# Kebii/MikuDance

Hardware: AMD Instinct MI355X
Metric: frames/sec (768x768, 16f, 20 DDIM steps) (higher is better)
Workload: dtype f16; 1 GPU; configs[1]: 768x768, 16-frame clip, 20 DDIM steps, fp16, reference_unet + denoising_unet + motion_module, CFG 3.5, one clip per GPU per step; parallelism=dp1, input_staging=rank-local (every rank stages its own clip in HBM before the timed region), reference_reuse=True, queues=1, weights=random-init SD-1.5 geometry (N(0,1/fan_in), seeds 1234/4321), width=full

## Files before the change

include/mdance_hip.h:

```cpp
#ifndef MDANCE_HIP_H
#define MDANCE_HIP_H
#include <stddef.h>
#ifdef __cplusplus
extern "C" {
#endif

#define MD_ACT_NONE 0
#define MD_ACT_SILU 1
#define MD_ACT_RELU 2
#define MD_ACT_GEGLU 3
#define MD_ACT_QUICKGELU 4

int md_version(void);
const char* md_last_error(void);

int md_gemm_f16(const void* A, int lda, const void* W, void* C, int ldc, int M, int N, int K, const void* bias,
                const void* residual, int ldr, const void* rowadd, int ldra, int rows_per_group, int act,
                int transpose_out, void* stream);

int md_conv3x3_nhwc_f16(const void* X, const void* W, void* Y, int ldy, int B, int Hin, int Win, int Cin, int Cout,
                        int stride, int upsample, const void* bias, const void* residual, int ldr,
                        const void* rowadd, int ldra, int rows_per_group, int act, void* stream);

int md_conv3x3_pad_nhwc_f16(const void* X, const void* W, void* Y, int ldy, int B, int Hin, int Win, int Cin, int Cout,
                            int stride, int upsample, int pad_lo, const void* bias, const void* residual, int ldr,
                            const void* rowadd, int ldra, int rows_per_group, int act, void* stream);

int md_conv_nhwc_f16(const void* X, int ldx, const void* W, void* Y, int ldy, int B, int Hin, int Win, int Cin, int Cout, int kw,
                     int stride, int upsample, int pad_lo, const void* bias, const void* residual, int ldr, const void* rowadd,
                     int ldra, int rows_per_group, int act, void* stream);

int md_softmax_rows_f16(void* x, int ldx, int rows, int cols, float scale, void* stream);

size_t md_groupnorm_workspace_bytes(int B, int HW, int C, int G);
int md_groupnorm_nhwc_f16(const void* x, void* y, const void* gamma, const void* beta, int B, int HW, int C, int G,
                          float eps, int silu, void* workspace, size_t ws_bytes, void* stream);

int md_groupnorm_ld_nhwc_f16(const void* x, int ldx, void* y, const void* gamma, const void* beta, int B, int HW, int C, int G,
                             float eps, int silu, void* workspace, size_t ws_bytes, void* stream);

int md_layernorm_f16(const void* x, void* y, void* y2, const void* gamma, const void* beta, const void* add, int M,
                     int C, float eps, int add_mode, int add_row_begin, int rows_per_frame, int frames, void* stream);

int md_groupnorm_plan(int B, int HW, int C, int G, int ldx, int x_align16, int table, int* threads, int* R, int* slab, int* nslab);

int md_layernorm_plan(int M, int C);

int md_gemm_ln_plan(int M, int N, int K, int act, int epi);
int md_gemm_ln_f16(const void* A, int lda, const void* Wf, const float* sc, void* C, int ldc, int M, int N, int K, float eps,
                   const void* rowadd, int ldra, int rows_per_group, int act, void* stream);

int md_groupnorm_table_f16(const void* x, int ldx, const void* gamma, const void* beta, int B, int HW, int C, int G, float eps,
                           float* table, void* workspace, size_t ws_bytes, void* stream);
int md_gemm_affine_plan(int M, int N, int K, int rows_per_image);
int md_gemm_affine_f16(const void* A, int lda, const float* table, int rows_per_image, const void* W, void* C, int ldc, int M, int N,
                       int K, const void* bias, void* stream);

int md_instnorm_spade_f16(const void* x, const void* gamma_beta, void* y, int B, int HW, int C, float eps,
                          void* stream);

int md_instnorm_spade_ld_f16(const void* x, int ldx, const void* gamma_beta, void* y, int B, int HW, int C, float eps,
                             void* stream);

int md_attention_fwd_f16(const void* Q, int ldq, const void* K, int ldk, const void* Vt, int ldvt, void* O, int ldo,
                         const int* kv_index, int B, int H, int D, int Lq, int Lk, int kv_stride, float scale,
                         void* stream);

int md_attention_plan(int D, int Lq, int Lk, int kv_stride, int ldvt, int vt_align16);

int md_temporal_attention_fwd_f16(const void* Q, int ldq, const void* K, int ldk, const void* V, int ldv, void* O,
                                  int ldo, int NB, int F, int HW, int H, int D, float scale, void* stream);

int md_temporal_attention_plan(int NB, int F, int HW, int H, int D, int aligned16, int* hg, int* pb);

int md_pack_nhwc_f16(const void* src, int src_is_f32, void* dst, int N, int F, long sB, long sF, long sC, long sY,
                     long sX, int c_begin, int c_count, int Cpad, int Ho, int Wo, int Hin, int Win, void* stream);
int md_unpack_nhwc_f16(const void* src, int ldc, void* dst, int dst_is_f32, int N, int F, long sB, long sF, long sC,
                       long sY, long sX, int C, int Ho, int Wo, void* stream);

int md_concat_channels_f16(const void* a, int Ca, const void* b, int Cb, void* out, long M, void* stream);

int md_window_accumulate(const void* pred, void* noise_sum, void* counter, const int* window, int f, int Ftot, int HW,
                         int halves, void* stream);

int md_window_accumulate_weighted(const void* pred, void* noise_sum, void* counter, const int* window, const float* weights, int f,
                                  int Ftot, int HW, int halves, void* stream);

int md_cfg_ddim_step(void* latents, const void* noise_sum, const void* counter, int Ftot, int HW, int halves,
                     float guidance, float alpha_t, float alpha_prev, void* stream);
// ... 84 lines not shown
```

mikudance_amd/_lib.py:

```python
import ctypes
import os
from ctypes import c_char_p, c_float, c_int, c_long, c_size_t, c_void_p

_HERE = os.path.dirname(os.path.abspath(__file__))
LIB_PATH = os.path.join(_HERE, "libmdance_hip.so")

P = c_void_p
SIGNATURES = {
    "md_version": (c_int, []),
    "md_last_error": (c_char_p, []),
    "md_gemm_f16": (c_int, [P, c_int, P, P, c_int, c_int, c_int, c_int, P, P, c_int, P, c_int, c_int, c_int, c_int, P]),
    "md_conv3x3_nhwc_f16": (c_int, [P, P, P, c_int, c_int, c_int, c_int, c_int, c_int, c_int, c_int, P, P, c_int, P, c_int,
                                    c_int, c_int, P]),
    "md_conv3x3_pad_nhwc_f16": (c_int, [P, P, P, c_int, c_int, c_int, c_int, c_int, c_int, c_int, c_int, c_int, P, P, c_int, P,
                                        c_int, c_int, c_int, P]),
    "md_conv_nhwc_f16": (c_int, [P, c_int, P, P, c_int, c_int, c_int, c_int, c_int, c_int, c_int, c_int, c_int, c_int, P, P, c_int, P,
                                 c_int, c_int, c_int, P]),
    "md_set_cu_limit": (c_int, [c_int]),
    "md_gemm_plan": (c_int, [c_int, c_int, c_int, c_int, c_int, c_int, c_int]),
    "md_conv3x3_plan": (c_int, [c_int, c_int, c_int, c_int, c_int, c_int, c_int, c_int, c_int]),
    "md_gemm_plan_call": (c_int, [P, c_int, P, P, c_int, c_int, c_int, c_int, P, P, c_int, P, c_int, c_int, c_int, c_int,
                                  ctypes.POINTER(c_int), ctypes.POINTER(c_int)]),
    "md_conv_plan_call": (c_int, [P, c_int, P, P, c_int, c_int, c_int, c_int, c_int, c_int, c_int, c_int, c_int, c_int, P, P, c_int, P,
                                  c_int, c_int, c_int]),
    "md_softmax_rows_f16": (c_int, [P, c_int, c_int, c_int, c_float, P]),
    "md_groupnorm_workspace_bytes": (c_size_t, [c_int, c_int, c_int, c_int]),
    "md_groupnorm_nhwc_f16": (c_int, [P, P, P, P, c_int, c_int, c_int, c_int, c_float, c_int, P, c_size_t, P]),
    "md_groupnorm_ld_nhwc_f16": (c_int, [P, c_int, P, P, P, c_int, c_int, c_int, c_int, c_float, c_int, P, c_size_t, P]),
    "md_instnorm_spade_ld_f16": (c_int, [P, c_int, P, P, c_int, c_int, c_int, c_float, P]),
    "md_layernorm_f16": (c_int, [P, P, P, P, P, P, c_int, c_int, c_float, c_int, c_int, c_int, c_int, P]),
    "md_groupnorm_plan": (c_int, [c_int, c_int, c_int, c_int, c_int, c_int, c_int] + [ctypes.POINTER(c_int)] * 4),
    "md_layernorm_plan": (c_int, [c_int, c_int]),
    "md_gemm_ln_plan": (c_int, [c_int, c_int, c_int, c_int, c_int]),
    "md_gemm_ln_f16": (c_int, [P, c_int, P, P, P, c_int, c_int, c_int, c_int, c_float, P, c_int, c_int, c_int, P]),
    "md_groupnorm_table_f16": (c_int, [P, c_int, P, P, c_int, c_int, c_int, c_int, c_float, P, P, c_size_t, P]),
    "md_gemm_affine_plan": (c_int, [c_int, c_int, c_int, c_int]),
    "md_gemm_affine_f16": (c_int, [P, c_int, P, c_int, P, P, c_int, c_int, c_int, c_int, P, P]),
    "md_instnorm_spade_f16": (c_int, [P, P, P, c_int, c_int, c_int, c_float, P]),
    "md_attention_fwd_f16": (c_int, [P, c_int, P, c_int, P, c_int, P, c_int, P, c_int, c_int, c_int, c_int, c_int, c_int,
                                     c_float, P]),
    "md_attention_plan": (c_int, [c_int, c_int, c_int, c_int, c_int, c_int]),
    "md_temporal_attention_fwd_f16": (c_int, [P, c_int, P, c_int, P, c_int, P, c_int, c_int, c_int, c_int, c_int, c_int,
                                              c_float, P]),
    "md_temporal_attention_plan": (c_int, [c_int, c_int, c_int, c_int, c_int, c_int, ctypes.POINTER(c_int), ctypes.POINTER(c_int)]),
    "md_pack_nhwc_f16": (c_int, [P, c_int, P, c_int, c_int, c_long, c_long, c_long, c_long, c_long, c_int, c_int, c_int,
                                 c_int, c_int, c_int, c_int, P]),
    "md_unpack_nhwc_f16": (c_int, [P, c_int, P, c_int, c_int, c_int, c_long, c_long, c_long, c_long, c_long, c_int, c_int,
                                   c_int, P]),
    "md_concat_channels_f16": (c_int, [P, c_int, P, c_int, P, c_long, P]),
    "md_window_accumulate": (c_int, [P, P, P, P, c_int, c_int, c_int, c_int, P]),
    "md_window_accumulate_weighted": (c_int, [P, P, P, P, P, c_int, c_int, c_int, c_int, P]),
    "md_cfg_ddim_step": (c_int, [P, P, P, c_int, c_int, c_int, c_float, c_float, c_float, P]),
    "md_cfg_ddim_step_eta": (c_int, [P, P, P, P, c_int, c_int, c_int, c_float, c_float, c_float, c_float, P]),
    "md_cfg_multistep_step": (c_int, [P, P, P, P, P, c_int, c_int, c_int, c_float, c_float, c_float, c_float, c_float, c_float, c_float, P]),
    "md_cfg_rescale_workspace_bytes": (c_size_t, [c_int, c_int]),
    "md_cfg_guidance_rescale": (c_int, [P, P, c_int, c_int, c_int, c_float, c_float, P, c_size_t, P, P]),
    "md_cfg_ddim_step_scaled": (c_int, [P, P, P, P, P, c_int, c_int, c_int, c_float, c_float, c_float, c_float, P]),
    "md_cfg_multistep_step_scaled": (c_int, [P, P, P, P, P, P, c_int, c_int, c_int, c_float, c_float, c_float, c_float, c_float, c_float,
                                             c_float, P]),
    "md_cfg_apg_workspace_bytes": (c_size_t, [c_int, c_int]),
    "md_cfg_apg_prepare": (c_int, [P, P, P, P, c_int, c_int, c_int, c_float, c_float, c_float, c_float, c_float, P, c_size_t, P, P]),
    "md_cfg_ddim_step_apg": (c_int, [P, P, P, P, P, P, c_int, c_int, c_int, c_float, c_float, c_float, c_float, P]),
    "md_cfg_multistep_step_apg": (c_int, [P, P, P, P, P, P, P, c_int, c_int, c_int, c_float, c_float, c_float, c_float, c_float, c_float,
                                          c_float, P]),
    "md_cfg_ddim_step_pag": (c_int, [P, P, P, P, P, c_int, c_int, c_int, c_float, c_float, c_float, c_float, c_float, P]),
    "md_cfg_multistep_step_pag": (c_int, [P, P, P, P, P, P, c_int, c_int, c_int, c_float, c_float, c_float, c_float, c_float, c_float, c_float,
                                          c_float, P]),
    "md_cfg_unipc_step": (c_int, [P, P, P, P, c_int, c_int, c_int, c_float, P, P]),
    "md_cfg_unipc_step_scaled": (c_int, [P, P, P, P, P, c_int, c_int, c_int, c_float, P, P]),
    "md_cfg_unipc_step_apg": (c_int, [P, P, P, P, P, P, c_int, c_int, c_int, c_float, P, P]),
# ... 80 lines not shown
```

mikudance_amd/blocks.py:

```python
from dataclasses import dataclass

import torch
from torch import nn

from . import ops, packing

GROUPS = 32
HEADS = 8


class _Packed(nn.Module):

    def __init__(self):
        super().__init__()
        self._pk = None

    def _apply(self, fn, *a, **k):
        self._pk = None
        return super()._apply(fn, *a, **k)

    def _load_from_state_dict(self, *a, **k):
        self._pk = None
        return super()._load_from_state_dict(*a, **k)

# ... 109 lines not shown
class _GEGLU(nn.Module):
    def __init__(self, dim):
        super().__init__()
        self.proj = Linear(dim, dim * 8)


class FeedForward(nn.Module):

    def __init__(self, dim):
        super().__init__()
        self.net = nn.ModuleList([_GEGLU(dim), nn.Identity(), Linear(dim * 4, dim)])


def _pack_ff(ff, dev, pk, prefix="ff"):
    w, b = packing.geglu_weight(ff.net[0].proj.weight, ff.net[0].proj.bias, dev)
    pk[prefix + "1"], pk[prefix + "1b"] = w, b
    pk[prefix + "2"], pk[prefix + "2b"] = packing.linear_weight(ff.net[2].weight, dev), packing.vec(ff.net[2].bias, dev)


FUSE_NORMS = __import__("os").environ.get("MD_FUSE_NORMS", "1") != "0"


def ln_linear(pk, h, norm, lin, bias=None, rowadd=None, rows_per_group=0, act=ops.ACT_NONE, eps=1e-5):
    M, K = h.shape
    w = pk[lin]
    if FUSE_NORMS and ops.gemm_ln_plan(M, w.shape[0], K, act, rowadd is not None, a=h):
        fk = lin + ":ln"
        if fk not in pk:
            pk[fk] = packing.ln_fold(w, None if bias is None else pk[bias], pk[norm + "w"], pk[norm + "b"])
        wf, sc = pk[fk]
        return ops.gemm_ln(h, wf, sc, eps=eps, rowadd=rowadd, rows_per_group=rows_per_group, act=act)
    n = ops.layernorm(h, pk[norm + "w"], pk[norm + "b"], eps=eps)
    return ops.gemm(n, w, bias=None if bias is None else pk[bias], rowadd=rowadd, rows_per_group=rows_per_group, act=act)


def gn_linear(x, gamma, beta, eps, w, bias):
    B, C = x.shape[0], x.shape[-1]
    M = x.numel() // C
    if FUSE_NORMS and ops.gemm_affine_plan(M, w.shape[0], C, M // B, x=x):
        return ops.gemm_affine(x, ops.groupnorm_table(x, gamma, beta, GROUPS, eps), w, bias=bias)
    return ops.gemm(tokens(ops.groupnorm(x, gamma, beta, GROUPS, eps)), w, bias=bias)


def _run_ff(pk, h, norm, prefix="ff"):
    g = ln_linear(pk, h, norm, prefix + "1", bias=prefix + "1b", act=ops.ACT_GEGLU)
    return ops.gemm(g, pk[prefix + "2"], bias=pk[prefix + "2b"], residual=h)


class CrossContext:

    def __init__(self, ctx, index, lk, lpad, zero_frames=0):
        self.ctx, self.index, self.lk, self.lpad = ctx, index, lk, lpad
        self.zero_frames = zero_frames
        self.root = self
        self._slices = {}

    def rows(self, lo, hi):
        s = self._slices.get((lo, hi))
        if s is None:
            s = CrossContext(self.ctx, self.index[lo:hi].contiguous(), self.lk, self.lpad, zero_frames=max(0, min(self.zero_frames, hi) - lo))
            s.root = self.root
            self._slices[(lo, hi)] = s
        return s


ZERO_CONTEXT_SKIP = True
# ... 15 lines not shown

    @property
    def perturbed(self):
        return self.identity is not None or self.blur is not None


PLAIN = SelfAttnCall()


class TransformerBlock(_Packed):

    def __init__(self, dim, ctx_dim, heads=HEADS, kind="2d"):
        super().__init__()
        self.dim, self.heads, self.kind = dim, heads, kind
        self.norm1 = Affine(dim)
        self.attn1 = Attention(dim)
        self.norm2 = Affine(dim)
        self.attn2 = Attention(dim, ctx_dim)
        self.norm3 = Affine(dim)
        self.ff = FeedForward(dim)
        self.bank = []
        self.ref_mode = None
        self.ref_cfg = False
        self.stop_after_bank = False
        self._kv_cache = None

    def _pack(self, dev):
        L, V = packing.linear_weight, packing.vec
        a1, a2 = self.attn1, self.attn2
        pk = {f"n{i}w": V(n.weight, dev) for i, n in ((1, self.norm1), (2, self.norm2), (3, self.norm3))}
        pk.update({f"n{i}b": V(n.bias, dev) for i, n in ((1, self.norm1), (2, self.norm2), (3, self.norm3))})
        pk["q1"], pk["k1"], pk["v1"] = L(a1.to_q.weight, dev), L(a1.to_k.weight, dev), L(a1.to_v.weight, dev)
        pk["qk1"] = torch.cat([pk["q1"], pk["k1"]], 0).contiguous()
        pk["o1"], pk["o1b"] = L(a1.to_out[0].weight, dev), V(a1.to_out[0].bias, dev)
        pk["q2"], pk["k2"], pk["v2"] = L(a2.to_q.weight, dev), L(a2.to_k.weight, dev), L(a2.to_v.weight, dev)
        pk["o2"], pk["o2b"] = L(a2.to_out[0].weight, dev), V(a2.to_out[0].bias, dev)
        _pack_ff(self.ff, dev, pk)
        self._kv_cache = None
        return pk

    def context_kv(self, cross):
        if self._kv_cache is None or self._kv_cache[0] is not cross.root:
            pk = self.packed()
            self._kv_cache = (cross.root, ops.gemm(cross.ctx, pk["k2"]), ops.gemm(cross.ctx, pk["v2"], transpose_out=True), {})
        return self._kv_cache[1:]

    def _self_attention(self, pk, n, kv, B, L, grid, sigma, pool, tile):
        C, H = self.dim, self.heads
        t, shift = tile or (1, None)
        th, tw = (grid[0] // t, grid[1] // t) if grid is not None else (None, None)
        Bt, Lt = (B, L) if tile is None else (B * t * t, th * tw)
        pad = None if tile is None else (Lt + 7) // 8 * 8

        def order(x, stride=None):
            return x if tile is None else ops.token_tile(x, B, grid[0], grid[1], t, shift, tile_stride=stride)[0]

        if n is kv and pool is None and sigma is None and pad in (None, Lt):
            src = order(n)
            qk = ops.gemm(src, pk["qk1"])
            q, k, Lk, stride = qk[:, :C], qk[:, C:], Lt, None
        else:
            if sigma is not None:
                q = order(ops.token_blur(ops.gemm(n, pk["q1"]), B, grid[0], grid[1], sigma))
            else:
                q = ops.gemm(order(n), pk["q1"])
            if pool is None:
                src, Lk, stride = order(kv, pad), Lt, pad
            else:
                src, Lk, stride = ops.token_pool(order(kv), Bt, th, tw, pool[0], pool[1])
            k = ops.gemm(src, pk["k1"])
        vt = ops.gemm(src, pk["v1"], transpose_out=True)
        a = ops.attention(q, k, vt, Bt, H, C // H, Lt, Lk, kv_stride=stride)
        return a if tile is None else ops.token_untile(a, B, grid[0], grid[1], t, shift)

    def forward(self, h, B, L, cross, sa=PLAIN, grid=None):
        pk = self.packed()
        C, H = self.dim, self.heads
        D = C // H
        if sa.perturbed and self.ref_mode == "write":
            raise ValueError("TransformerBlock: a perturbed evaluation is a call of its own: not a bank write")
        identity = sa.identity is not None and any(self is b for b in sa.identity)
        sigma = sa.blur[1] if sa.blur is not None and any(self is b for b in sa.blur[0]) else None
        pool = None if sa.pool is None or identity else sa.pool.get(self)
        tile = None if sa.tile is None or identity else sa.tile.get(self)
        if (sigma is not None or pool is not None or tile is not None) and (grid is None or grid[0] * grid[1] != L):
            raise ValueError(f"TransformerBlock: grid {grid} does not hold L = {L} tokens")
        M = h.shape[0]
        if self.ref_mode != "read" or len(self.bank) != 1 or (self.ref_cfg and sa.half == 0):
            begin = None
        elif sa.perturbed or sa.half == 1 or not self.ref_cfg:
            begin = 0
        else:
            begin = M // 2
        if begin is None:
            n = kv = ops.layernorm(h, pk["n1w"], pk["n1b"])
            if self.ref_mode == "write":
                self.bank.append(n.view(B, L, C))
                if self.stop_after_bank:
                    return h
        else:
            b2 = self.bank[0].reshape(-1, C)
            if (self.ref_cfg or sa.perturbed) and b2.shape[0] == 2 * (M - begin):
                b2 = b2[M - begin:]
            assert b2.shape[0] == M - begin, (b2.shape, M)
# ... 168 lines not shown
```

mikudance_amd/csrc/gemm.hip:

```cpp
#include "common.h"
#include <stdlib.h>
#include <algorithm>


enum { ACT_NONE = 0, ACT_SILU = 1, ACT_RELU = 2, ACT_GEGLU = 3, ACT_QUICKGELU = 4 };

struct GemmParams {
  const half_t* A;
  const half_t* W;
  half_t* C;
  const half_t* bias;
  const half_t* residual;
  const half_t* rowadd;
  int lda, ldc, ldr, ldra;
  int M, N, K;
  int rows_per_group;
  int act;
  int transpose_out;
  int bias_rows;
  int Hin, Win, Cin, Hout, Wout, stride, upsample, pad;
  int ldx;
  int kw;
  int tiles_n, tiles_total;
  int tiles_m, group_m;
// ... 564 lines not shown
  MD_CHECK_LAUNCH("md_gemm_ln");
  return MD_OK;
}

extern "C" int md_gemm_affine_plan(int M, int N, int K, int rows_per_image) {
  return rows_per_image > 0 && rows_per_image % 16 == 0 && M % rows_per_image == 0 && ws_fused_shape(M, N, K, K, N);
}

extern "C" int md_gemm_affine_f16(const void* A, int lda, const float* table, int rows_per_image, const void* W, void* C, int ldc, int M, int N,
                                  int K, const void* bias, void* stream) {
  MD_CHECK_ARG(rows_per_image > 0 && rows_per_image % 16 == 0 && M % rows_per_image == 0 && ws_fused_shape(M, N, K, lda, ldc),
               "md_gemm_affine: no fused kernel for M=%d N=%d K=%d rows_per_image=%d (ask md_gemm_affine_plan first)", M, N, K, rows_per_image);
  MD_CHECK_ARG(al16(A) && al16(W) && al16(C) && al16(table) && al16(bias), "md_gemm_affine: operands must be 16-byte aligned");
  MD_CHECK_ARG(A != C, "md_gemm_affine: in place is not supported");
  WsParams p = {};
  p.A = (const half_t*)A; p.W = (const half_t*)W; p.C = (half_t*)C; p.bias = (const half_t*)bias;
  p.lda = lda; p.ldc = ldc; p.M = M; p.N = N; p.rows_per_group = 1;
  p.aff = table; p.rows_per_image = rows_per_image;
  p.groups = N / 320; ws_streams(p);
  hipStream_t st = (hipStream_t)stream;
  if (p.groups > 1) launch_ws_fused<2, false, PRO_AFF>(p, st);
  else launch_ws_fused<1, false, PRO_AFF>(p, st);
  MD_CHECK_LAUNCH("md_gemm_affine");
  return MD_OK;
}

static bool ws_eligible(const GemmParams& p) {
  if (p.act != ACT_NONE || p.transpose_out || p.M < 32768 || p.M % 16) return false;
  const bool k320 = p.K == 320 && p.N % 320 == 0 && p.N / 320 <= 8;
  const bool k640 = p.K == 640 && p.N % 128 == 0 && p.N / 128 <= 16;
  if (!k320 && !k640) return false;
  if (p.lda % 8 || p.ldc % 8 || (p.residual && p.ldr % 8) || (p.rowadd && p.ldra % 8)) return false;
  return al16(p.A) && al16(p.W) && al16(p.C) && al16(p.bias) && al16(p.residual) && al16(p.rowadd);
}

struct SpTile {
  int code, bm, bn;
  double t_k;
  int pin;
  bool (*eligible)(const GemmParams&);
  bool (*resm)(const GemmParams&);
  void (*launch)(GemmParams&, bool resm, int ncu, hipStream_t);
};
template <bool CONV, bool GEGLU, int MT, int NT>
static SpTile sp_tile(double t_k, int pin) {
  return {100 + 10 * MT + NT, 64 * MT, 64 * NT, t_k, pin, sp_eligible<CONV, GEGLU, NT>, GEGLU ? nullptr : sp_resm<MT, NT>,
          launch_sp<CONV, GEGLU, NT, MT>};
}
enum { T135, T134, T124, T142, T132, T144, SP_TILES };
static const SpTile& sp_tiles(bool conv, int t) {
  static const double tk32 = md_env_int("MD_GEMM_SP_TK32", 800) * 1e-3;
  static const SpTile rows[2][SP_TILES] = {
      {sp_tile<false, false, 3, 5>(1.56, 5), sp_tile<false, false, 3, 4>(1.28, 4), sp_tile<false, false, 2, 4>(0.95, 2),
       sp_tile<false, false, 4, 2>(0.95, 42), sp_tile<false, false, 3, 2>(tk32, 32), sp_tile<false, true, 4, 4>(0, 0)},
      {sp_tile<true, false, 3, 5>(1.56, 5), sp_tile<true, false, 3, 4>(1.28, 4), sp_tile<true, false, 2, 4>(0.95, 2),
       sp_tile<true, false, 4, 2>(0.95, 42), sp_tile<true, false, 3, 2>(tk32, 32), {}}};
  return rows[conv][t];
}

static long sp_tile_count(const SpTile& t, const GemmParams& p) { return (long)cdiv(p.M, t.bm) * (p.N / t.bn); }
static double sp_cost(const SpTile& t, const GemmParams& p, int ncu) {
  return (double)cdiv(sp_tile_count(t, p), ncu) * (4.0 + (p.K / 64) * t.t_k);
}

static GemmParams gemm_swapped(const GemmParams& p) {
  GemmParams q = p;
// ... 286 lines not shown
```

mikudance_amd/csrc/gemm_ws.h:

```cpp
#pragma once
#ifndef WS_ABL
#define WS_ABL 0
#endif
#ifndef WS_RES_DEPTH
#define WS_RES_DEPTH 4
#endif
#ifndef WS_RES_DEPTH_640
#define WS_RES_DEPTH_640 8
#endif

struct WsParams {
  const half_t* A;
  const half_t* W;
  half_t* C;
  const half_t* bias;
  const half_t* residual;
  const half_t* rowadd;
  int lda, ldc, ldr, ldra;
  int M, N;
  int rows_per_group;
  int groups;
  int streams;
  int spx;
  int xstreams;
  const float* lnf;
  float eps;
  const float* aff;
  int rows_per_image;
};

enum { PRO_NONE = 0, PRO_LNF = 1, PRO_AFF = 2 };

template <int KS, int CB, int TPR>
struct WsCfg {
  static constexpr int K = 32 * KS;
  static constexpr int CPR = K / 8;
  static constexpr int GC = 64 * CB;
  static constexpr int TR = 16;
  static constexpr int STAGE = TR * K * 2;
  static constexpr int RSTAGE = TPR * STAGE;
  static constexpr bool GEGLU_CFG = CB == 4;
  static constexpr int CS_LD = GC + 4;
  static constexpr int CSTAGE = TR * CS_LD * 4;
  static constexpr int OSTAGE = GEGLU_CFG ? 2 * 2048 : 0;
  static constexpr int SSLOT = TR;
  static constexpr int SSTAGE = 4 * TPR * SSLOT * 8;
  static constexpr int NR_FIT = (160 * 1024 - 2 * TPR * CSTAGE - OSTAGE - SSTAGE) / RSTAGE;
  static constexpr int NR = NR_FIT > 12 ? 12 : NR_FIT;
  static constexpr int DPT = STAGE / 1024;
  static constexpr int PER = DPT / 2;
  static constexpr int SMEM = NR * RSTAGE + 2 * TPR * CSTAGE + OSTAGE + SSTAGE;
  static constexpr int CHUNKS = TR * GC / 8;
  static constexpr int SPL = CHUNKS / 128;
  static constexpr int PD = KS <= 10 ? 3 : 6;
  static_assert(DPT % 2 == 0 && CHUNKS % 128 == 0, "tile must split evenly over the loader / store waves");
  static_assert(NR >= 3 && (NR - 2) * TPR * PER <= 63, "ring depth / vmcnt immediate");
  static constexpr int RES_DEPTH = KS == 20 ? WS_RES_DEPTH_640 : WS_RES_DEPTH;
  static_assert(RES_DEPTH % TPR == 0, "residual buffers are indexed statically per unrolled round");
};

__device__ __forceinline__ float ws_sum8(float v) {
// ... 4 lines not shown
}

template <int CPR>
__device__ __forceinline__ int ws_swz(int row) {
  return CPR == 40 ? ((row >> 1) & 7) : (row & 15);
}

struct WsGegluPiece {
  int row, hcol;
  float bh[8], bg[8];
};
__device__ __forceinline__ half8_t ws_geglu_piece(const float* cs, int cs_ld, const WsGegluPiece& q) {
  const float* s = cs + q.row * cs_ld + q.hcol;
  const floatx4 h0 = *reinterpret_cast<const floatx4*>(s), h1 = *reinterpret_cast<const floatx4*>(s + 4);
  const floatx4 g0 = *reinterpret_cast<const floatx4*>(s + 32), g1 = *reinterpret_cast<const floatx4*>(s + 36);
  half8_t o;
  float2_t gl[4];
#pragma unroll
  for (int j = 0; j < 2; ++j) {
    gl[j] = float2_t{g0[2 * j] + q.bg[2 * j], g0[2 * j + 1] + q.bg[2 * j + 1]};
    gl[j + 2] = float2_t{g1[2 * j] + q.bg[2 * j + 4], g1[2 * j + 1] + q.bg[2 * j + 5]};
  }
  gelu_fast2_x<4>(gl);
#pragma unroll
  for (int j = 0; j < 2; ++j) {
    o[2 * j] = (half_t)((h0[2 * j] + q.bh[2 * j]) * gl[j].x);
    o[2 * j + 1] = (half_t)((h0[2 * j + 1] + q.bh[2 * j + 1]) * gl[j].y);
    o[2 * j + 4] = (half_t)((h1[2 * j] + q.bh[2 * j + 4]) * gl[j + 2].x);
    o[2 * j + 5] = (half_t)((h1[2 * j + 1] + q.bh[2 * j + 5]) * gl[j + 2].y);
  }
  return o;
}

template <int KS, int CB, int TPR, bool RES, bool RA, bool GEGLU = false, int PRO = PRO_NONE>
__global__ __launch_bounds__(512, 1) void wsgemm_kernel(WsParams p) {
  constexpr bool LN = PRO == PRO_LNF;
  static_assert(PRO == PRO_NONE || !GEGLU, "GEGLU has no prologue flavour: its memory waves are VALU bound by the GELU");
  static_assert(!GEGLU || (CB == 4 && TPR == 1 && !RES && !RA), "GEGLU: 2 h + 2 g column blocks per compute wave, one tile per round, bias only");
  static_assert(PRO == PRO_NONE || !RES, "prologue flavours: no residual (their consumers have none)");

  static_assert(PRO != PRO_AFF || (!RA && !GEGLU), "PRO_AFF: bias only");
  using Cfg = WsCfg<KS, CB, TPR>;
  auto lslot_of = [](int r, int u) { return ((r & 3) * TPR + u) * Cfg::SSLOT; };
  constexpr int K = Cfg::K, CPR = Cfg::CPR, GC = Cfg::GC, TR = Cfg::TR, STAGE = Cfg::STAGE, RSTAGE = Cfg::RSTAGE, NR = Cfg::NR,
                CS_LD = Cfg::CS_LD;
  extern __shared__ __attribute__((aligned(16))) char smem[];
  char* ring = smem;
  float* cst = reinterpret_cast<float*>(smem + NR * RSTAGE);
  char* ost = smem + NR * RSTAGE + 2 * TPR * Cfg::CSTAGE;
  float2_t* lst = reinterpret_cast<float2_t*>(smem + NR * RSTAGE + 2 * TPR * Cfg::CSTAGE + Cfg::OSTAGE);
  const int tid = threadIdx.x, wave = tid >> 6, lane = tid & 63;
  const int xcd = blockIdx.x & 7, slot = blockIdx.x >> 3;
  int grp = slot % p.groups, stream = xcd * p.spx + slot / p.groups;
  if (slot >= p.groups * p.spx) {
    const int left = 32 - p.groups * p.spx, e = xcd * left + (slot - p.groups * p.spx);
    if (e >= p.xstreams * p.groups) return;
    grp = e % p.groups;
    stream = 8 * p.spx + e / p.groups;
  }
  const int ntiles = (p.M + TR - 1) / TR;
  const int tps = (ntiles + p.streams - 1) / p.streams;
  const int tile0 = PRO == PRO_AFF ? stream * tps : stream;
  const int tstep = PRO == PRO_AFF ? 1 : p.streams;
  const int my_tiles = PRO == PRO_AFF ? max(0, min(tps, ntiles - tile0)) : (stream < ntiles ? (ntiles - stream + p.streams - 1) / p.streams : 0);
  if (my_tiles == 0) return;
  const int rounds = (my_tiles + TPR - 1) / TPR;
  const int n0 = grp * GC;
  WsGegluPiece gp = {};
  if constexpr (GEGLU) {
    if (wave >= 4) {
      const int id = (wave - 4) * 64 + lane;
      gp.row = id / (GC / 16);
      const int oc = (id % (GC / 16)) * 8;
      gp.hcol = 64 * (oc >> 5) + (oc & 31);
      {
        const half8_t b0 = p.bias ? *reinterpret_cast<const half8_t*>(p.bias + n0 + gp.hcol) : half8_t{0, 0, 0, 0, 0, 0, 0, 0};
        const half8_t b1 = p.bias ? *reinterpret_cast<const half8_t*>(p.bias + n0 + gp.hcol + 32) : half8_t{0, 0, 0, 0, 0, 0, 0, 0};
#pragma unroll
        for (int j = 0; j < 8; ++j) gp.bh[j] = (float)b0[j], gp.bg[j] = (float)b1[j];
      }
    }
  }

  if (wave < 4) {
    half8_t wf[CB][KS];
    {
      const half_t* wp = p.W + (size_t)(n0 + wave * 16 * CB + (lane & 15)) * K + 8 * (lane >> 4);
#pragma unroll
      for (int cb = 0; cb < CB; ++cb)
#pragma unroll
        for (int ks = 0; ks < KS; ++ks) wf[cb][ks] = *reinterpret_cast<const half8_t*>(wp + (size_t)cb * 16 * K + 32 * ks);
    }
    const int row = lane & 15, kq = lane >> 4;
    const int rbase = row * CPR, sw = ws_swz<CPR>(row);
    __builtin_amdgcn_s_waitcnt(0x0F70);
    constexpr int PD = Cfg::PD;
    constexpr int SWB = CPR == 40 ? 3 : 4, P = (1 << SWB) / 4;
// ... 181 lines not shown
        }
        if (r >= 1 && r <= rounds) {
          *reinterpret_cast<half8_t*>(cp_own) = ws_geglu_piece(cst + ((r - 1) & 1) * (TR * CS_LD), CS_LD, gp);
          cp_own += cstep;
        }
      }
    } else {
      const int sid = (wave - 6) * 64 + lane;
      constexpr int CPRO = GC / 8;
      constexpr int SPL = Cfg::SPL;
      int prow[SPL], pcol[SPL];
      float biasf[SPL][8];
      half_t* cp[SPL];
      const half_t* rp[SPL];
      const size_t cstep = (size_t)tstep * TR * p.ldc, rstep = (size_t)tstep * TR * p.ldr;
      float lsf[LN ? SPL : 1][8], lcf[LN ? SPL : 1][8];
#pragma unroll
      for (int i = 0; i < SPL; ++i) {
        const int id = i * 128 + sid;
        prow[i] = id / CPRO;
        pcol[i] = (id % CPRO) * 8;
        const half8_t bv = p.bias ? *reinterpret_cast<const half8_t*>(p.bias + n0 + pcol[i]) : half8_t{0, 0, 0, 0, 0, 0, 0, 0};
#pragma unroll
        for (int j = 0; j < 8; ++j) biasf[i][j] = (float)bv[j];
        cp[i] = p.C + (size_t)(tile0 * TR + prow[i]) * p.ldc + n0 + pcol[i];
        rp[i] = RES ? p.residual + (size_t)(tile0 * TR + prow[i]) * p.ldr + n0 + pcol[i] : nullptr;
        if constexpr (LN) {
          const floatx4 s0 = *reinterpret_cast<const floatx4*>(p.lnf + n0 + pcol[i]), s1 = *reinterpret_cast<const floatx4*>(p.lnf + n0 + pcol[i] + 4);
          const floatx4 c0 = *reinterpret_cast<const floatx4*>(p.lnf + p.N + n0 + pcol[i]), c1 = *reinterpret_cast<const floatx4*>(p.lnf + p.N + n0 + pcol[i] + 4);
#pragma unroll
          for (int j = 0; j < 4; ++j) lsf[i][j] = s0[j], lsf[i][j + 4] = s1[j], lcf[i][j] = c0[j], lcf[i][j + 4] = c1[j];
        }
      }
#ifndef WS_PRE_WAIT
#define WS_PRE_WAIT 1
#endif
      if constexpr (WS_PRE_WAIT) __builtin_amdgcn_s_waitcnt(0x0F70);
      constexpr int RD = RA ? (KS == 20 ? 4 : 2) : Cfg::RES_DEPTH;
      static_assert(RD % TPR == 0, "residual buffers are indexed statically per unrolled round");
      constexpr int UNR = RD / TPR;
      half8_t res[RES ? RD : 1][SPL];
      int cur_group = -1;
      float raf[RA ? SPL : 1][8];
      auto store_tile = [&](int tile, int buf, int lslot, const half8_t (&rs)[SPL]) {
        const int m0 = (tile0 + tile * tstep) * TR;
        const float* cs = cst + buf * (TR * CS_LD);
#if WS_ABL & 8
        return;
#endif
        if constexpr (RA) {
          const int g0 = m0 / p.rows_per_group, g1 = (m0 + TR - 1) / p.rows_per_group;
          if (g0 != cur_group || g1 != g0) {
#pragma unroll
            for (int i = 0; i < SPL; ++i) {
              const int g = g1 == g0 ? g0 : (m0 + prow[i]) / p.rows_per_group;
              const half8_t ra = *reinterpret_cast<const half8_t*>(p.rowadd + (size_t)g * p.ldra + n0 + pcol[i]);
#pragma unroll
              for (int j = 0; j < 8; ++j) raf[i][j] = (float)ra[j];
            }
            __builtin_amdgcn_s_waitcnt(0x0F70);
            cur_group = g1 == g0 ? g0 : -1;
          }
        }
        floatx4 ca[SPL], cb2[SPL];
        float2_t ab[LN ? SPL : 1];
#pragma unroll
        for (int i = 0; i < SPL; ++i) {
          ca[i] = *reinterpret_cast<const floatx4*>(cs + prow[i] * CS_LD + pcol[i]);
          cb2[i] = *reinterpret_cast<const floatx4*>(cs + prow[i] * CS_LD + pcol[i] + 4);
          if constexpr (LN) ab[i] = lst[lslot + prow[i]];
        }
#pragma unroll
        for (int i = 0; i < SPL; ++i) {
          float v[8] = {ca[i][0], ca[i][1], ca[i][2], ca[i][3], cb2[i][0], cb2[i][1], cb2[i][2], cb2[i][3]};
          if constexpr (LN) {
#pragma unroll
            for (int j = 0; j < 8; ++j) v[j] = ab[i].x * v[j] + (ab[i].y * lsf[i][j] + lcf[i][j]);
          } else {
#pragma unroll
            for (int j = 0; j < 8; ++j) v[j] += biasf[i][j];
          }
          if constexpr (RA) {
// ... 102 lines not shown
```

mikudance_amd/ops.py:

```python
import ctypes

import torch

from . import _lib

ACT_NONE, ACT_SILU, ACT_RELU, ACT_GEGLU, ACT_QUICKGELU = 0, 1, 2, 3, 4
F16 = torch.float16


def _st():
    return torch.cuda.current_stream().cuda_stream


def _p(t):
    return 0 if t is None else t.data_ptr()


def _chk(t, name, dtype=F16):
    if t is None:
        return
    if not t.is_cuda:
        raise _lib.MdanceHipError(f"{name} must live on the GPU: mikudance_amd has no CPU path")
    if t.dtype != dtype:
        raise _lib.MdanceHipError(f"{name} must be {dtype}, got {t.dtype}")
# ... 31 lines not shown
    _chk(w, "w")
    M, K = a.shape
    N = w.shape[0]
    assert w.shape[1] == K and w.is_contiguous(), (w.shape, K)
    if out is None:
        if transpose_out:
            out = torch.empty((N, ldc_t or M), device=a.device, dtype=F16)
        else:
            out = torch.empty((M, N // 2 if act == ACT_GEGLU else N), device=a.device, dtype=F16)
    ldc = _rowmajor(out, "out")
    ldr = _rowmajor(residual, "residual") if residual is not None else 0
    ldra = _rowmajor(rowadd, "rowadd") if rowadd is not None else 0
    _chk(bias, "bias")
    return (a.data_ptr(), lda, w.data_ptr(), out.data_ptr(), ldc, M, N, K, _p(bias), _p(residual), ldr, _p(rowadd), ldra, rows_per_group,
            act, int(transpose_out)), out


def gemm(a, w, bias=None, residual=None, rowadd=None, rows_per_group=0, act=ACT_NONE, transpose_out=False, out=None,
         ldc_t=None):
    args, out = _gemm_args(a, w, bias, residual, rowadd, rows_per_group, act, transpose_out, out, ldc_t)
    M, N, K = args[5:8]
    _lib.call("md_gemm_f16", *args, _st(),
              meta=(f"gemm M={M} N={N} K={K}" + (" geglu" if act == ACT_GEGLU else "") + (" T" if transpose_out else ""),
                    2.0 * M * N * K, 2.0 * (M * K + N * K + M * N)))
    return out


def gemm_plan(a, w, bias=None, residual=None, rowadd=None, rows_per_group=0, act=ACT_NONE, transpose_out=False, out=None,
              ldc_t=None, blocks=False):
    args, _ = _gemm_args(a, w, bias, residual, rowadd, rows_per_group, act, transpose_out, out, ldc_t)
    nb, tail = ctypes.c_int(1), ctypes.c_int(0)
    code = _lib.load().md_gemm_plan_call(*args, ctypes.byref(nb), ctypes.byref(tail))
    return (code, nb.value, tail.value) if blocks else code


def _conv_args(x, w, cout, bias, residual, rowadd, rows_per_group, act, stride, upsample, out, pad_lo, kw):
    _chk(w, "w")
    assert x.dim() == 4
    ldx = _pixel_pitch(x, "x")
    B, H, W, Cin = x.shape
    assert w.shape == (cout, 3 * kw * Cin) and w.is_contiguous(), (w.shape, cout, Cin)
    hup, wup = (H * 2, W * 2) if upsample else (H, W)
    Ho, Wo = (hup + pad_lo - 2) // stride + 1, ((wup + pad_lo - 2) // stride + 1 if kw == 3 else W)
    if out is None:
        out = torch.empty((B, Ho, Wo, cout), device=x.device, dtype=F16)
    assert tuple(out.shape) == (B, Ho, Wo, cout), (tuple(out.shape), (B, Ho, Wo, cout))
    ldy = _pixel_pitch(out, "out", align=1)
    r2 = residual.flatten(0, -2) if residual is not None else None
    ldr = _rowmajor(r2, "residual") if r2 is not None else 0
    ldra = _rowmajor(rowadd, "rowadd") if rowadd is not None else 0
    _chk(bias, "bias")
    return (x.data_ptr(), ldx, w.data_ptr(), out.data_ptr(), ldy, B, H, W, Cin, cout, kw, stride, int(upsample), int(pad_lo), _p(bias),
            _p(r2), ldr, _p(rowadd), ldra, rows_per_group, act), out, (Ho, Wo)


def conv3x3(x, w, cout, bias=None, residual=None, rowadd=None, rows_per_group=0, act=ACT_NONE, stride=1, upsample=False,
            out=None, pad_lo=1, kw=3):
    args, out, (Ho, Wo) = _conv_args(x, w, cout, bias, residual, rowadd, rows_per_group, act, stride, upsample, out, pad_lo, kw)
    B, H, W, Cin = x.shape
    _lib.call("md_conv_nhwc_f16", *args, _st(),
              meta=(f"conv3x{kw} B={B} {H}x{W} Cin={Cin} Cout={cout} s={stride} up={int(upsample)}",
                    2.0 * B * Ho * Wo * cout * 3 * kw * Cin, 2.0 * (B * H * W * Cin + cout * 3 * kw * Cin + B * Ho * Wo * cout)))
    return out


def conv_plan(x, w, cout, bias=None, residual=None, rowadd=None, rows_per_group=0, act=ACT_NONE, stride=1, upsample=False,
# ... 500 lines not shown
```

Baseline: 7.335 frames/s.

## Fuse K/V projections with transposed V output into one warp-specialized GEMM

Adds a split-epilogue mode to the warp-specialized GEMM. Columns below n_split are stored row-major, and the remaining columns are written transposed into a separate Vt buffer. Self-attention now issues a single GEMM (QKV or KV concatenated weights) instead of two, so the activation matrix is read once instead of twice and one launch is saved. The fused path is restricted to large M with K of 320 or 640. It can be disabled through an environment variable, and it adds a transposed-store epilogue whose memory efficiency is uncertain.

```diff
diff --git a/include/mdance_hip.h b/include/mdance_hip.h
--- a/include/mdance_hip.h
+++ b/include/mdance_hip.h
@@ -55,6 +55,10 @@
 int md_gemm_affine_plan(int M, int N, int K, int rows_per_image);
 int md_gemm_affine_f16(const void* A, int lda, const float* table, int rows_per_image, const void* W, void* C, int ldc, int M, int N,
                        int K, const void* bias, void* stream);
+
+int md_gemm_split_t_plan(int M, int N, int K, int n_split, int lda, int ldc, int ldct);
+int md_gemm_split_t_f16(const void* A, int lda, const void* W, void* C, int ldc, void* Ct, int ldct, int M, int N, int K, int n_split,
+                        void* stream);
 
 int md_instnorm_spade_f16(const void* x, const void* gamma_beta, void* y, int B, int HW, int C, float eps,
                           void* stream);
diff --git a/mikudance_amd/_lib.py b/mikudance_amd/_lib.py
--- a/mikudance_amd/_lib.py
+++ b/mikudance_amd/_lib.py
@@ -36,6 +36,8 @@
     "md_groupnorm_table_f16": (c_int, [P, c_int, P, P, c_int, c_int, c_int, c_int, c_float, P, P, c_size_t, P]),
     "md_gemm_affine_plan": (c_int, [c_int, c_int, c_int, c_int]),
     "md_gemm_affine_f16": (c_int, [P, c_int, P, c_int, P, P, c_int, c_int, c_int, c_int, P, P]),
+    "md_gemm_split_t_plan": (c_int, [c_int, c_int, c_int, c_int, c_int, c_int, c_int]),
+    "md_gemm_split_t_f16": (c_int, [P, c_int, P, P, c_int, P, c_int, c_int, c_int, c_int, c_int, P]),
     "md_instnorm_spade_f16": (c_int, [P, P, P, c_int, c_int, c_int, c_float, P]),
     "md_attention_fwd_f16": (c_int, [P, c_int, P, c_int, P, c_int, P, c_int, P, c_int, c_int, c_int, c_int, c_int, c_int,
                                      c_float, P]),
diff --git a/mikudance_amd/blocks.py b/mikudance_amd/blocks.py
--- a/mikudance_amd/blocks.py
+++ b/mikudance_amd/blocks.py
@@ -165,6 +165,15 @@
         return ops.gemm_ln(h, wf, sc, eps=eps, rowadd=rowadd, rows_per_group=rows_per_group, act=act)
     n = ops.layernorm(h, pk[norm + "w"], pk[norm + "b"], eps=eps)
     return ops.gemm(n, w, bias=None if bias is None else pk[bias], rowadd=rowadd, rows_per_group=rows_per_group, act=act)
+
+
+FUSE_KVT = __import__("os").environ.get("MD_FUSE_KVT", "1") != "0"
+
+
+def kv_t(src, w, w_plain, w_t):
+    if FUSE_KVT and ops.gemm_split_t_plan(src, w, w_plain.shape[0]):
+        return ops.gemm_split_t(src, w, w_plain.shape[0])
+    return ops.gemm(src, w_plain), ops.gemm(src, w_t, transpose_out=True)
 
 
 def gn_linear(x, gamma, beta, eps, w, bias):
@@ -246,6 +255,8 @@
         pk.update({f"n{i}b": V(n.bias, dev) for i, n in ((1, self.norm1), (2, self.norm2), (3, self.norm3))})
         pk["q1"], pk["k1"], pk["v1"] = L(a1.to_q.weight, dev), L(a1.to_k.weight, dev), L(a1.to_v.weight, dev)
         pk["qk1"] = torch.cat([pk["q1"], pk["k1"]], 0).contiguous()
+        pk["kv1"] = torch.cat([pk["k1"], pk["v1"]], 0).contiguous()
+        pk["qkv1"] = torch.cat([pk["qk1"], pk["v1"]], 0).contiguous()
         pk["o1"], pk["o1b"] = L(a1.to_out[0].weight, dev), V(a1.to_out[0].bias, dev)
         pk["q2"], pk["k2"], pk["v2"] = L(a2.to_q.weight, dev), L(a2.to_k.weight, dev), L(a2.to_v.weight, dev)
         pk["o2"], pk["o2b"] = L(a2.to_out[0].weight, dev), V(a2.to_out[0].bias, dev)
@@ -271,7 +282,7 @@
 
         if n is kv and pool is None and sigma is None and pad in (None, Lt):
             src = order(n)
-            qk = ops.gemm(src, pk["qk1"])
+            qk, vt = kv_t(src, pk["qkv1"], pk["qk1"], pk["v1"])
             q, k, Lk, stride = qk[:, :C], qk[:, C:], Lt, None
         else:
             if sigma is not None:
@@ -282,8 +293,7 @@
                 src, Lk, stride = order(kv, pad), Lt, pad
             else:
                 src, Lk, stride = ops.token_pool(order(kv), Bt, th, tw, pool[0], pool[1])
-            k = ops.gemm(src, pk["k1"])
-        vt = ops.gemm(src, pk["v1"], transpose_out=True)
+            k, vt = kv_t(src, pk["kv1"], pk["k1"], pk["v1"])
         a = ops.attention(q, k, vt, Bt, H, C // H, Lt, Lk, kv_stride=stride)
         return a if tile is None else ops.token_untile(a, B, grid[0], grid[1], t, shift)
 
diff --git a/mikudance_amd/csrc/gemm.hip b/mikudance_amd/csrc/gemm.hip
--- a/mikudance_amd/csrc/gemm.hip
+++ b/mikudance_amd/csrc/gemm.hip
@@ -620,6 +620,50 @@
   if (!k320 && !k640) return false;
   if (p.lda % 8 || p.ldc % 8 || (p.residual && p.ldr % 8) || (p.rowadd && p.ldra % 8)) return false;
   return al16(p.A) && al16(p.W) && al16(p.C) && al16(p.bias) && al16(p.residual) && al16(p.rowadd);
+}
+
+static int ws_split_group(int K) { return K == 320 ? 320 : (K == 640 ? 128 : 0); }
+
+static int ws_split_code(int M, int N, int K, int n_split, int lda, int ldc, int ldct) {
+  MD_CHECK_ARG(M > 0 && N > 0 && K > 0 && n_split > 0 && n_split < N, "md_gemm_split_t: need 0 < n_split=%d < N=%d (M=%d K=%d)", n_split, N, M, K);
+  MD_CHECK_ARG(lda >= K && ldc >= n_split && ldct >= M, "md_gemm_split_t: lda=%d / ldc=%d / ldct=%d must cover K=%d / n_split=%d / M=%d", lda, ldc,
+               ldct, K, n_split, M);
+  const int gc = ws_split_group(K);
+  if (!gc || M < 32768 || M % 16 || N % gc || N / gc > (K == 320 ? 8 : 16)) return 0;
+  MD_CHECK_ARG(lda % 8 == 0 && ldc % 8 == 0, "md_gemm_split_t: lda=%d / ldc=%d must be multiples of 8 (16-byte pieces)", lda, ldc);
+  MD_CHECK_ARG(ldct % 8 == 0, "md_gemm_split_t: ldct=%d must be a multiple of 8 (16-byte stores along the token axis)", ldct);
+  MD_CHECK_ARG(n_split % gc == 0, "md_gemm_split_t: n_split=%d must be a multiple of the column-group width %d of K=%d", n_split, gc, K);
+  return K == 320 ? 210 : 220;
+}
+
+extern "C" int md_gemm_split_t_plan(int M, int N, int K, int n_split, int lda, int ldc, int ldct) {
+  return ws_split_code(M, N, K, n_split, lda, ldc, ldct);
+}
+
+template <int KS, int CB>
+static void launch_ws_split(const WsParams& p, hipStream_t stream) {
+  using Cfg = WsCfg<KS, CB, 2>;
+  md_ensure_dynamic_lds<wsgemm_kernel<KS, CB, 2, false, false, false, PRO_NONE, true>>(Cfg::SMEM);
+  hipLaunchKernelGGL((wsgemm_kernel<KS, CB, 2, false, false, false, PRO_NONE, true>), dim3(256), dim3(512), Cfg::SMEM, stream, p);
+}
+
+extern "C" int md_gemm_split_t_f16(const void* A, int lda, const void* W, void* C, int ldc, void* Ct, int ldct, int M, int N, int K, int n_split,
+                                   void* stream) {
+  const int code = ws_split_code(M, N, K, n_split, lda, ldc, ldct);
+  if (code < 0) return code;
+  MD_CHECK_ARG(code > 0, "md_gemm_split_t: no fused kernel for M=%d N=%d K=%d (ask md_gemm_split_t_plan first)", M, N, K);
+  MD_CHECK_ARG(A && W && C && Ct && al16(A) && al16(W) && al16(C) && al16(Ct), "md_gemm_split_t: operands must be 16-byte aligned");
+  static const int contig_env = md_env_int("MD_WS_SPLIT_CONTIG", -1);
+  const int contig = contig_env < 0 ? K == 640 : contig_env;
+  WsParams p = {};
+  p.A = (const half_t*)A; p.W = (const half_t*)W; p.C = (half_t*)C; p.Ct = (half_t*)Ct;
+  p.lda = lda; p.ldc = ldc; p.ldct = ldct; p.n_split = n_split; p.contig = contig; p.M = M; p.N = N; p.rows_per_group = 1;
+  p.groups = N / ws_split_group(K);
+  ws_streams(p);
+  if (code == 210) launch_ws_split<10, 5>(p, (hipStream_t)stream);
+  else launch_ws_split<20, 2>(p, (hipStream_t)stream);
+  MD_CHECK_LAUNCH("md_gemm_split_t");
+  return MD_OK;
 }
 
 struct SpTile {
diff --git a/mikudance_amd/csrc/gemm_ws.h b/mikudance_amd/csrc/gemm_ws.h
--- a/mikudance_amd/csrc/gemm_ws.h
+++ b/mikudance_amd/csrc/gemm_ws.h
@@ -27,6 +27,9 @@
   float eps;
   const float* aff;
   int rows_per_image;
+  half_t* Ct;
+  int ldct, n_split;
+  int contig;
 };
 
 enum { PRO_NONE = 0, PRO_LNF = 1, PRO_AFF = 2 };
@@ -97,8 +100,9 @@
   return o;
 }
 
-template <int KS, int CB, int TPR, bool RES, bool RA, bool GEGLU = false, int PRO = PRO_NONE>
+template <int KS, int CB, int TPR, bool RES, bool RA, bool GEGLU = false, int PRO = PRO_NONE, bool SPLIT = false>
 __global__ __launch_bounds__(512, 1) void wsgemm_kernel(WsParams p) {
+  static_assert(!SPLIT || (!RES && !RA && !GEGLU && PRO == PRO_NONE), "SPLIT: plain epilogue only");
   constexpr bool LN = PRO == PRO_LNF;
   static_assert(PRO == PRO_NONE || !GEGLU, "GEGLU has no prologue flavour: its memory waves are VALU bound by the GELU");
   static_assert(!GEGLU || (CB == 4 && TPR == 1 && !RES && !RA), "GEGLU: 2 h + 2 g column blocks per compute wave, one tile per round, bias only");
@@ -125,9 +129,10 @@
   }
   const int ntiles = (p.M + TR - 1) / TR;
   const int tps = (ntiles + p.streams - 1) / p.streams;
-  const int tile0 = PRO == PRO_AFF ? stream * tps : stream;
-  const int tstep = PRO == PRO_AFF ? 1 : p.streams;
-  const int my_tiles = PRO == PRO_AFF ? max(0, min(tps, ntiles - tile0)) : (stream < ntiles ? (ntiles - stream + p.streams - 1) / p.streams : 0);
+  const bool contig = PRO == PRO_AFF || (SPLIT && p.contig);
+  const int tile0 = contig ? stream * tps : stream;
+  const int tstep = contig ? 1 : p.streams;
+  const int my_tiles = contig ? max(0, min(tps, ntiles - tile0)) : (stream < ntiles ? (ntiles - stream + p.streams - 1) / p.streams : 0);
   if (my_tiles == 0) return;
   const int rounds = (my_tiles + TPR - 1) / TPR;
   const int n0 = grp * GC;
@@ -375,6 +380,18 @@
           for (int j = 0; j < 4; ++j) lsf[i][j] = s0[j], lsf[i][j + 4] = s1[j], lcf[i][j] = c0[j], lcf[i][j + 4] = c1[j];
         }
       }
+      const bool tr = SPLIT && n0 >= p.n_split;
+      const int th = sid & 1;
+      int toff[SPLIT ? SPL : 1];
+      half_t* ctp[SPLIT ? SPL : 1];
+      if constexpr (SPLIT) {
+#pragma unroll
+        for (int i = 0; i < SPL; ++i) {
+          const int tcol = (i * 128 + sid) >> 1;
+          toff[i] = 12 * th * CS_LD + tcol;
+          ctp[i] = tr ? p.Ct + (size_t)(n0 - p.n_split + tcol) * p.ldct + (size_t)tile0 * TR + 8 * th : nullptr;
+        }
+      }
 #ifndef WS_PRE_WAIT
 #define WS_PRE_WAIT 1
 #endif
@@ -391,6 +408,30 @@
 #if WS_ABL & 8
         return;
 #endif
+        if constexpr (SPLIT) {
+          if (tr) {
+            float t[SPL][8];
+#pragma unroll
+            for (int i = 0; i < SPL; ++i) {
+              const float* a = cs + toff[i];
+              const float* b = a + (4 - 8 * th) * CS_LD;
+#pragma unroll
+              for (int j = 0; j < 4; ++j) t[i][j] = a[j * CS_LD], t[i][j + 4] = b[j * CS_LD];
+            }
+#pragma unroll
+            for (int i = 0; i < SPL; ++i) {
+              half8_t o;
+#pragma unroll
+              for (int j = 0; j < 4; ++j) {
+                o[j] = (half_t)(th ? t[i][j + 4] : t[i][j]);
+                o[j + 4] = (half_t)(th ? t[i][j] : t[i][j + 4]);
+              }
+              *reinterpret_cast<half8_t*>(ctp[i]) = o;
+              ctp[i] += (size_t)tstep * TR;
+            }
+            return;
+          }
+        }
         if constexpr (RA) {
           const int g0 = m0 / p.rows_per_group, g1 = (m0 + TR - 1) / p.rows_per_group;
           if (g0 != cur_group || g1 != g0) {
diff --git a/mikudance_amd/ops.py b/mikudance_amd/ops.py
--- a/mikudance_amd/ops.py
+++ b/mikudance_amd/ops.py
@@ -87,6 +87,48 @@
     nb, tail = ctypes.c_int(1), ctypes.c_int(0)
     code = _lib.load().md_gemm_plan_call(*args, ctypes.byref(nb), ctypes.byref(tail))
     return (code, nb.value, tail.value) if blocks else code
+
+
+def _split_t_dims(a, w, n_split, out, out_t, ldc_t, launch=True):
+    def pitch(t, name):
+        if launch:
+            return _rowmajor(t, name)
+        if t.dim() != 2 or t.stride(1) != 1:
+            raise _lib.MdanceHipError(f"{name} must be a 2-D row-major matrix (stride(1) == 1)")
+        return t.stride(0)
+    lda = pitch(a, "a")
+    if launch:
+        _chk(w, "w")
+    M, K = a.shape
+    N = w.shape[0]
+    assert w.shape[1] == K and w.is_contiguous(), (w.shape, K)
+    ldc = pitch(out, "out") if out is not None else n_split
+    ldct = pitch(out_t, "out_t") if out_t is not None else (ldc_t or M)
+    return M, N, K, lda, ldc, ldct
+
+
+def gemm_split_t_plan(a, w, n_split, out=None, out_t=None, ldc_t=None):
+    M, N, K, lda, ldc, ldct = _split_t_dims(a, w, n_split, out, out_t, ldc_t, launch=False)
+    lib = _lib.load()
+    code = lib.md_gemm_split_t_plan(M, N, K, n_split, lda, ldc, ldct)
+    if code < 0:
+        raise _lib.MdanceHipError(f"md_gemm_split_t_plan failed ({code}): {lib.md_last_error().decode()}")
+    if code and not all(t is None or t.is_meta or t.data_ptr() % 16 == 0 for t in (a, w, out, out_t)):
+        return 0
+    return code
+
+
+def gemm_split_t(a, w, n_split, out=None, out_t=None, ldc_t=None):
+    M, N, K, lda, ldc, ldct = _split_t_dims(a, w, n_split, out, out_t, ldc_t)
+    if out is None:
+        out = torch.empty((M, n_split), device=a.device, dtype=F16)
+    if out_t is None:
+        out_t = torch.empty((N - n_split, ldct), device=a.device, dtype=F16)
+    if tuple(out.shape) != (M, n_split) or out_t.shape[0] != N - n_split or out_t.shape[1] < M:
+        raise _lib.MdanceHipError(f"gemm_split_t: out {tuple(out.shape)} / out_t {tuple(out_t.shape)} do not fit M={M} N={N} n_split={n_split}")
+    _lib.call("md_gemm_split_t_f16", a.data_ptr(), lda, w.data_ptr(), out.data_ptr(), ldc, out_t.data_ptr(), ldct, M, N, K, n_split, _st(),
+              meta=(f"gemm M={M} N={N} K={K} kT", 2.0 * M * N * K, 2.0 * (M * K + N * K + M * N)))
+    return out, out_t
 
 
 def _conv_args(x, w, cout, bias, residual, rowadd, rows_per_group, act, stride, upsample, out, pad_lo, kw):
```

Result: no change. 7.365 frames/s, median of 6 (+0.4%).
